# Haiga/nn-with-pytorch-personalized-losses

Hardware: AMD Instinct MI355X
Metric: slates/sec fwd+bwd approxNDCG slate=128 feat=136 (higher is better)
Workload: dtype f32; 1 GPU; approxNDCG + doubleLayerNet (136-136-136-1) train-mode dropout, 100000 queries x slate 128 x 136 feat fp32 per GPU resident in HBM, 25000 slates per GPU per step, one fused launch (fwd+loss+bwd) + grad all-reduce + Adam; queries_per_gpu=100000, slate=128, features=136, batch_per_gpu=25000, net=double, step_windows=4, step_windows_visited=4, last_window_starts_at_float=1305600000, parallelism=query-sharded dp1

## Files before the change

nn-with-pytorch-personalized-losses_amd/csrc/ltr_scorer.hip:

```cpp
#include "../../include/ltr_mi355x.h"
#include "ltr_slate_losses.h"
#include <math.h>
#include <stdlib.h>
#include <string.h>
#include <type_traits>


#ifndef LTR_F16X2
#define LTR_F16X2 0
#endif
#ifndef LTR_LOLO
#define LTR_LOLO 1
#endif

using namespace ltr;

typedef float f32x4 __attribute__((ext_vector_type(4)));

namespace {

constexpr int kTileDocs = 128;
constexpr int kWaves = 8;
constexpr int kThreads = kWaves * 64;
constexpr int kChunkDocs = 64;
// ... 298 lines not shown
                v = __frcp_rn(1.f + __expf(-v))      ;
            }
            if (16 * To + 16 > H) v = (16 * To + 4 * q + r < H) ? v : 0.f;
            h[To][r] = v;
        }
    }
}

template <int ACT>
__device__ __forceinline__ float apply_act_grad(float g, float h) {
    if (ACT == ACT_RELU_DROP) return h > 0.f ? g : 0.f;
    if (ACT == ACT_SIGMOID) return g * (h * (1.f - h));
    return g;
}

template <int NR, int NC, int BH>
__host__ __device__ constexpr int dw_row(int g) { return (g / (NC * BH)) * BH + (g % (NC * BH)) % BH; }
template <int NR, int NC, int BH>
__host__ __device__ constexpr int dw_col(int g) { return (g % (NC * BH)) / BH; }
__host__ __device__ constexpr int dw_count(int NW, int W) {
    const int s = W % (kWaves / 2), simd = NW / (kWaves / 2) + (s < NW % (kWaves / 2) ? 1 : 0);
    return W < kWaves / 2 ? (simd + 1) / 2 : simd / 2;
}
__host__ __device__ constexpr int dw_first(int NW, int W) {
    int g = 0;
    for (int v = 0; v < W; ++v) g += dw_count(NW, v);
    return g;
}
__host__ __device__ constexpr bool dw_sets_balanced(int NW) {
    const int TW = (NW + kWaves - 1) / kWaves;
    int lo = NW, hi = 0;
    for (int s = 0; s < kWaves / 2; ++s) {
        const int t = dw_count(NW, s) + dw_count(NW, s + kWaves / 2);
        lo = t < lo ? t : lo;
        hi = t > hi ? t : hi;
        if (dw_count(NW, s) > TW || dw_count(NW, s + kWaves / 2) > TW) return false;
    }
    return hi - lo <= 1 && dw_first(NW, kWaves) == NW;
}

template <int W, int TW, int NR, int NC, int BH>
struct DwSet {
    static_assert(dw_sets_balanced(NR * NC) && TW == (NR * NC + kWaves - 1) / kWaves, "unbalanced dW tile sets");
    static constexpr int first = dw_first(NR * NC, W), count = dw_count(NR * NC, W);
    static constexpr bool uses_row(int To) {
        for (int j = 0; j < count; ++j)
            if (dw_row<NR, NC, BH>(first + j) == To) return true;
        return false;
    }
    static constexpr bool uses_col(int Ti) {
        for (int j = 0; j < count; ++j)
            if (dw_col<NR, NC, BH>(first + j) == Ti) return true;
        return false;
    }
    static constexpr int n_frags() {
        int n = 0;
        for (int t = 0; t < NR; ++t) n += uses_row(t) ? 1 : 0;
        for (int t = 0; t < NC; ++t) n += uses_col(t) ? 1 : 0;
        return n;
    }
    static constexpr int n_tiles() { return count; }
};

template <int W, int TW, int NR, int NC, int BH, int LD>
__device__ __forceinline__ void dw_load(float (&af)[NR], float (&bf)[NC], const float *ar, const float *br) {
#pragma unroll
    for (int To = 0; To < NR; ++To)
        if (DwSet<W, TW, NR, NC, BH>::uses_row(To)) af[To] = ar[16 * To];
#pragma unroll
    for (int Ti = 0; Ti < NC; ++Ti)
        if (DwSet<W, TW, NR, NC, BH>::uses_col(Ti)) bf[Ti] = br[16 * Ti];
}

template <int W, int TW, int NR, int NC, int BH>
__device__ __forceinline__ void dw_mfma(f32x4 (&acc)[TW], const float (&af)[NR], const float (&bf)[NC]) {
#pragma unroll
    for (int j = 0; j < DwSet<W, TW, NR, NC, BH>::count; ++j) {
        const int g = DwSet<W, TW, NR, NC, BH>::first + j;
        acc[j] = mfma4(af[dw_row<NR, NC, BH>(g)], bf[dw_col<NR, NC, BH>(g)], acc[j]);
    }
}

#ifndef LTR_DW_PIPE
#define LTR_DW_PIPE 0
#endif
#ifndef LTR_PRIO
#define LTR_PRIO 0
#endif
#ifndef LTR_KROT
#define LTR_KROT 0
#endif
#ifndef LTR_H1_BITS
#define LTR_H1_BITS 0
#endif
#ifndef LTR_STG_SWZ
#define LTR_STG_SWZ 0
#endif

template <int W, int TW, int NR, int NC, int BH, int LD>
__device__ __forceinline__ void dw_chunk_w(f32x4 (&acc)[TW], const float *a_base, const float *b_base, const float *a_odd,
                                           const float *b_odd) {
    constexpr int KS = kChunkDocs / 4;
#if LTR_DW_PIPE
    static_assert(!LTR_STG_SWZ, "the pipelined variant reads unswizzled images");
    constexpr int NF = DwSet<W, TW, NR, NC, BH>::n_frags();
    constexpr int NM = DwSet<W, TW, NR, NC, BH>::n_tiles();
    float af0[NR], bf0[NC], af1[NR], bf1[NC];
    dw_load<W, TW, NR, NC, BH, LD>(af0, bf0, a_base, b_base);
#pragma unroll
    for (int s = 0; s < KS; s += 2) {
        dw_load<W, TW, NR, NC, BH, LD>(af1, bf1, a_base + (s + 1) * 4 * LD, b_base + (s + 1) * 4 * LD);
        dw_mfma<W, TW, NR, NC, BH>(acc, af0, bf0);
#pragma unroll
        for (int i = 0; i < (NM > NF ? NM : NF); ++i) {
            if (i < NF) __builtin_amdgcn_sched_group_barrier(0x100, 1, 0);
            if (i < NM) __builtin_amdgcn_sched_group_barrier(0x008, 1, 0);
        }
        if (s + 2 < KS)
            dw_load<W, TW, NR, NC, BH, LD>(af0, bf0, a_base + (s + 2) * 4 * LD, b_base + (s + 2) * 4 * LD);
        dw_mfma<W, TW, NR, NC, BH>(acc, af1, bf1);
#pragma unroll
        for (int i = 0; i < (NM > NF ? NM : NF); ++i) {
            if (i < NF && s + 2 < KS) __builtin_amdgcn_sched_group_barrier(0x100, 1, 0);
            if (i < NM) __builtin_amdgcn_sched_group_barrier(0x008, 1, 0);
        }
    }
#else
    for (int s0 = 0; s0 < KS; ++s0) {
        const int s = LTR_KROT ? ((s0 + (W >= kWaves / 2 ? KS / 2 : 0)) % KS) : s0;
        float af[NR], bf[NC];
        dw_load<W, TW, NR, NC, BH, LD>(af, bf, ((s & 1) ? a_odd : a_base) + s * 4 * LD, ((s & 1) ? b_odd : b_base) + s * 4 * LD);
        dw_mfma<W, TW, NR, NC, BH>(acc, af, bf);
    }
#endif
}

template <int TW, int NR, int NC, int BH, int LD>
__device__ __forceinline__ void dw_chunk(int w, f32x4 (&acc)[TW], const float *a_base, const float *b_base, const float *a_odd = nullptr,
                                         const float *b_odd = nullptr) {
    if (!a_odd) a_odd = a_base;
    if (!b_odd) b_odd = b_base;
    switch (w) {
        case 0: dw_chunk_w<0, TW, NR, NC, BH, LD>(acc, a_base, b_base, a_odd, b_odd); break;
        case 1: dw_chunk_w<1, TW, NR, NC, BH, LD>(acc, a_base, b_base, a_odd, b_odd); break;
        case 2: dw_chunk_w<2, TW, NR, NC, BH, LD>(acc, a_base, b_base, a_odd, b_odd); break;
        case 3: dw_chunk_w<3, TW, NR, NC, BH, LD>(acc, a_base, b_base, a_odd, b_odd); break;
        case 4: dw_chunk_w<4, TW, NR, NC, BH, LD>(acc, a_base, b_base, a_odd, b_odd); break;
        case 5: dw_chunk_w<5, TW, NR, NC, BH, LD>(acc, a_base, b_base, a_odd, b_odd); break;
        case 6: dw_chunk_w<6, TW, NR, NC, BH, LD>(acc, a_base, b_base, a_odd, b_odd); break;
        default: dw_chunk_w<7, TW, NR, NC, BH, LD>(acc, a_base, b_base, a_odd, b_odd); break;
    }
}

#if LTR_F16X2
typedef short s16x4 __attribute__((ext_vector_type(4)));
typedef _Float16 h16x4 __attribute__((ext_vector_type(4)));
typedef unsigned int u32x2 __attribute__((ext_vector_type(2)));

template <int LDH>
__device__ __forceinline__ h16x8 tr_frag_h(const uint16_t *lane_base, int r0, int t) {
    typedef __attribute__((address_space(3))) s16x4 *lp4;
    const uint16_t *p = lane_base + r0 * LDH + 16 * t;
    const s16x4 lo = __builtin_amdgcn_ds_read_tr16_b64_v4i16((lp4)(p));
    const s16x4 hi = __builtin_amdgcn_ds_read_tr16_b64_v4i16((lp4)(p + 16 * LDH));
    const u32x2 l2 = __builtin_bit_cast(u32x2, lo), h2 = __builtin_bit_cast(u32x2, hi);
    return __builtin_bit_cast(h16x8, u32x4{l2[0], l2[1], h2[0], h2[1]});
}

__device__ __forceinline__ void split4(const f32x4 &v, float sc, u32x2 &hi, u32x2 &lo) {
    h16x4 h, l;
#pragma unroll
    for (int r = 0; r < 4; ++r) {
        const float x = v[r] * sc;
        h[r] = (_Float16)x;
        l[r] = (_Float16)(x - (float)h[r]);
    }
    hi = __builtin_bit_cast(u32x2, h);
    lo = __builtin_bit_cast(u32x2, l);
}

template <int W, int TW, int NR, int NC, int BH, int LDH, int KS>
__device__ __forceinline__ void dw_chunk_h_w(f32x4 (&acc)[TW], const uint16_t *ahi, const uint16_t *alo, const uint16_t *bhi,
                                             const uint16_t *blo) {
    using S = DwSet<W, TW, NR, NC, BH>;
#pragma unroll
    for (int s = 0; s < KS; ++s) {
        h16x8 ah[NR], al[NR];
#pragma unroll
        for (int To = 0; To < NR; ++To)
            if (S::uses_row(To)) {
                ah[To] = tr_frag_h<LDH>(ahi, 32 * s, To);
                al[To] = tr_frag_h<LDH>(alo, 32 * s, To);
            }
#pragma unroll
        for (int Ti = 0; Ti < NC; ++Ti)
            if (S::uses_col(Ti)) {
                const h16x8 bh = tr_frag_h<LDH>(bhi, 32 * s, Ti), bl = tr_frag_h<LDH>(blo, 32 * s, Ti);
#pragma unroll
                for (int j = 0; j < S::count; ++j) {
                    const int g = S::first + j;
                    if (dw_col<NR, NC, BH>(g) == Ti) {
                        const int r = dw_row<NR, NC, BH>(g);
                        acc[j] = __builtin_amdgcn_mfma_f32_16x16x32_f16(ah[r], bh, acc[j], 0, 0, 0);
                        acc[j] = __builtin_amdgcn_mfma_f32_16x16x32_f16(ah[r], bl, acc[j], 0, 0, 0);
                        acc[j] = __builtin_amdgcn_mfma_f32_16x16x32_f16(al[r], bh, acc[j], 0, 0, 0);
                        if (LTR_LOLO) acc[j] = __builtin_amdgcn_mfma_f32_16x16x32_f16(al[r], bl, acc[j], 0, 0, 0);
                    }
                }
            }
    }
}

template <int TW, int NR, int NC, int BH, int LDH, int KS>
__device__ __forceinline__ void dw_chunk_h(int w, f32x4 (&acc)[TW], const uint16_t *ahi, const uint16_t *alo, const uint16_t *bhi,
                                           const uint16_t *blo) {
    switch (w) {
        case 0: dw_chunk_h_w<0, TW, NR, NC, BH, LDH, KS>(acc, ahi, alo, bhi, blo); break;
        case 1: dw_chunk_h_w<1, TW, NR, NC, BH, LDH, KS>(acc, ahi, alo, bhi, blo); break;
        case 2: dw_chunk_h_w<2, TW, NR, NC, BH, LDH, KS>(acc, ahi, alo, bhi, blo); break;
        case 3: dw_chunk_h_w<3, TW, NR, NC, BH, LDH, KS>(acc, ahi, alo, bhi, blo); break;
        case 4: dw_chunk_h_w<4, TW, NR, NC, BH, LDH, KS>(acc, ahi, alo, bhi, blo); break;
        case 5: dw_chunk_h_w<5, TW, NR, NC, BH, LDH, KS>(acc, ahi, alo, bhi, blo); break;
        case 6: dw_chunk_h_w<6, TW, NR, NC, BH, LDH, KS>(acc, ahi, alo, bhi, blo); break;
        default: dw_chunk_h_w<7, TW, NR, NC, BH, LDH, KS>(acc, ahi, alo, bhi, blo); break;
    }
}

template <int NT, int KT, int LDH, int NMAX>
__device__ __forceinline__ void gemm_wx_hx(__amdgpu_buffer_rsrc_t rsrc, int base_bytes, int lane_off, const uint16_t *xhi_row,
                                           const uint16_t *xlo_row, f32x4 (&out)[NMAX], float un) {
    constexpr int KP = (KT + 1) / 2;
    constexpr int NSTEP = KP * NT, NLOAD = 2 * NSTEP, R = LTR_RING_H;
    f32x4 ring[R];
#pragma unroll
    for (int n = 0; n < R; ++n)
        if (n < NLOAD) ring[n] = load_frag(rsrc, lane_off, base_bytes + n * 1024);
#pragma unroll
    for (int To = 0; To < NT; ++To) out[To] = f32x4{0.f, 0.f, 0.f, 0.f};
    h16x8 bhi, blo;
#pragma unroll
    for (int n = 0; n < NSTEP; ++n) {
        const int P = n / NT, To = n % NT;
        if (To == 0) {
            const u32x2 z = {0u, 0u};
            const u32x2 h0 = *reinterpret_cast<const u32x2 *>(xhi_row + 32 * P), l0 = *reinterpret_cast<const u32x2 *>(xlo_row + 32 * P);
            const u32x2 h1 = 2 * P + 1 < KT ? *reinterpret_cast<const u32x2 *>(xhi_row + 32 * P + 16) : z;
            const u32x2 l1 = 2 * P + 1 < KT ? *reinterpret_cast<const u32x2 *>(xlo_row + 32 * P + 16) : z;
            bhi = __builtin_bit_cast(h16x8, u32x4{h0[0], h0[1], h1[0], h1[1]});
            blo = __builtin_bit_cast(h16x8, u32x4{l0[0], l0[1], l1[0], l1[1]});
        }
        const h16x8 ahi = __builtin_bit_cast(h16x8, ring[(2 * n) % R]);
        const h16x8 alo = __builtin_bit_cast(h16x8, ring[(2 * n + 1) % R]);
        if (2 * n + R < NLOAD) ring[(2 * n) % R] = load_frag(rsrc, lane_off, base_bytes + (2 * n + R) * 1024);
        if (2 * n + 1 + R < NLOAD) ring[(2 * n + 1) % R] = load_frag(rsrc, lane_off, base_bytes + (2 * n + 1 + R) * 1024);
        out[To] = __builtin_amdgcn_mfma_f32_16x16x32_f16(ahi, bhi, out[To], 0, 0, 0);
        out[To] = __builtin_amdgcn_mfma_f32_16x16x32_f16(ahi, blo, out[To], 0, 0, 0);
        out[To] = __builtin_amdgcn_mfma_f32_16x16x32_f16(alo, bhi, out[To], 0, 0, 0);
        if (LTR_LOLO) out[To] = __builtin_amdgcn_mfma_f32_16x16x32_f16(alo, blo, out[To], 0, 0, 0);
        __builtin_amdgcn_sched_barrier(0);
    }
#pragma unroll
    for (int To = 0; To < NT; ++To) out[To] *= un;
}

__device__ __forceinline__ int grow_exp(int ex, float m) {
    int e = __builtin_amdgcn_frexp_expf(m);
    e = m > 0.f ? e : -100;
    e = e < -100 ? -100 : e;
    return e > ex ? e : ex;
}
#endif

template <int W, int TW, int NR, int NC, int BH>
__device__ __forceinline__ void dw_store_w(const f32x4 (&acc)[TW], float *dst, int q, int d, float scale) {
#pragma unroll
    for (int j = 0; j < DwSet<W, TW, NR, NC, BH>::count; ++j) {
        const int g = DwSet<W, TW, NR, NC, BH>::first + j;
        const int To = dw_row<NR, NC, BH>(g), Ti = dw_col<NR, NC, BH>(g);
#pragma unroll
        for (int r = 0; r < 4; ++r) dst[(16 * To + 4 * q + r) * (NC * 16) + 16 * Ti + d] = acc[j][r] * scale;
    }
}

template <int TW, int NR, int NC, int BH>
__device__ __forceinline__ void dw_store(int w, const f32x4 (&acc)[TW], float *dst, int q, int d, float scale = 1.f) {
    switch (w) {
        case 0: dw_store_w<0, TW, NR, NC, BH>(acc, dst, q, d, scale); break;
        case 1: dw_store_w<1, TW, NR, NC, BH>(acc, dst, q, d, scale); break;
        case 2: dw_store_w<2, TW, NR, NC, BH>(acc, dst, q, d, scale); break;
        case 3: dw_store_w<3, TW, NR, NC, BH>(acc, dst, q, d, scale); break;
        case 4: dw_store_w<4, TW, NR, NC, BH>(acc, dst, q, d, scale); break;
        case 5: dw_store_w<5, TW, NR, NC, BH>(acc, dst, q, d, scale); break;
        case 6: dw_store_w<6, TW, NR, NC, BH>(acc, dst, q, d, scale); break;
        default: dw_store_w<7, TW, NR, NC, BH>(acc, dst, q, d, scale); break;
    }
}

#ifdef LTR_STAMPS
#define LTR_STAMP(k)                                                                                          \
    if (a.stamps && lane == 0 && (st - (int)blockIdx.x) / (int)gridDim.x == a.stamp_tile)                      \
        a.stamps[((size_t)blockIdx.x * kWaves + w) * 16 + (k)] = __builtin_readcyclecounter();
#else
#define LTR_STAMP(k)
#endif

template <class N>
__host__ __device__ constexpr int kXV4() { return (16 * (N::F / 4) + 63) / 64; }

template <class N>
__device__ __forceinline__ void load_x_tile(f32x4 (&xr)[kXV4<N>()], const PipeArgs &a, long long row0, int lane) {
    constexpr int V4_PER_ROW = N::F / 4;
    constexpr int V4 = 16 * V4_PER_ROW;
    const f32x4 *src = reinterpret_cast<const f32x4 *>(a.X + row0 * N::F);
#pragma unroll
    for (int m = 0; m < kXV4<N>(); ++m) {
        const int e = lane + 64 * m;
        f32x4 v = {0.f, 0.f, 0.f, 0.f};
        if (e < V4 && row0 + e / V4_PER_ROW < a.n_docs) v = src[e];
        xr[m] = v;
    }
}

#ifndef LTR_LOSS_UNR
#define LTR_LOSS_UNR 1
#endif
#ifndef LTR_XDMA
#define LTR_XDMA 1
#endif
#ifndef LTR_PIPE_ST128_MAXH
#define LTR_PIPE_ST128_MAXH 64
#endif
#ifndef LTR_PIPE_ST128
#define LTR_PIPE_ST128 1
#endif
#ifndef LTR_X_AUX
#define LTR_X_AUX 2
#endif
template <class N>
__device__ __forceinline__ void dma_x_rows(const PipeArgs &a, float *Xs, long long row0, int w, int lane) {
    typedef __attribute__((address_space(1))) const void *gptr_t;
    typedef __attribute__((address_space(3))) void *lptr_t;
#pragma unroll
    for (int r = 0; r < 16; ++r) {
        float *dst = Xs + (16 * w + r) * N::LD;
        if (row0 + r < a.n_docs) {
            if (lane < N::F / 4)
                __builtin_amdgcn_global_load_lds((gptr_t)(a.X + (row0 + r) * N::F + 4 * lane), (lptr_t)dst, 16, 0, LTR_X_AUX);
        } else if (lane < N::F / 4) {
            *reinterpret_cast<f32x4 *>(dst + 4 * lane) = f32x4{0.f, 0.f, 0.f, 0.f};
        }
    }
}

template <class N, class Stamp>
__device__ __forceinline__ void dw2_chunks(int w, int chunk, int crow, int q, int d, const f32x4 (&dz2)[N::NT2], const f32x4 (&h1)[N::H1T],
                                           f32x4 (&acc)[N::TW2], float *Ds, float *Hs, Stamp stamp) {
    constexpr int LD = N::LD;
#pragma unroll
    for (int c = 0; c < 2; ++c) {
        if (c > 0) __syncthreads();
        if (chunk == c) {
#pragma unroll
            for (int To = 0; To < N::NT2; ++To)
                *reinterpret_cast<f32x4 *>(Ds + crow * LD + 16 * To + ((4 * q) ^ (LTR_STG_SWZ ? 4 * ((crow >> 1) & 3) : 0))) = dz2[To];
#pragma unroll
            for (int T = 0; T < N::H1T; ++T)
                *reinterpret_cast<f32x4 *>(Hs + crow * LD + 16 * T + ((4 * q) ^ (LTR_STG_SWZ ? 4 * ((crow >> 1) & 3) : 0))) = h1[T];
        }
#ifdef LTR_STAMPS_DW
        stamp(c == 0 ? 10 : 13);
#endif
        __syncthreads();
#ifdef LTR_STAMPS_DW
        stamp(c == 0 ? 11 : 14);
#endif
        dw_chunk<N::TW2, N::NT2, N::H1T, N::BH2, LD>(w, acc, Ds + q * LD + (d ^ (LTR_STG_SWZ ? 4 * (q >> 1) : 0)),
                                                     Hs + q * LD + (d ^ (LTR_STG_SWZ ? 4 * (q >> 1) : 0)),
                                                     Ds + q * LD + (d ^ (LTR_STG_SWZ ? 4 * (2 + (q >> 1)) : 0)),
                                                     Hs + q * LD + (d ^ (LTR_STG_SWZ ? 4 * (2 + (q >> 1)) : 0)));
#ifdef LTR_STAMPS_DW
        if (c == 0) stamp(12);
#endif
    }
}

#include "ltr_fcw.h"

template <class N, int MODE, int LOSS, int ST = 0>
__global__ void __launch_bounds__(kThreads, 2) slate_pipeline_kernel(const PipeArgs a) {
    constexpr int LD = N::LD;
    extern __shared__ __attribute__((aligned(16))) float smem[];
    float *Xs = smem;
    float *Ds = Xs + kTileDocs * LD;
    float *Hs = Ds + kChunkDocs * LD;
    float *sc = Hs + kChunkDocs * LD;
    float *yl = sc + kTileDocs;
    float *gn = yl + kTileDocs;
    float *gg = gn + kTileDocs;
    float *dsc = gg + kTileDocs;
    float *uu = dsc + kTileDocs;
    float *mk = uu + kTileDocs;
    float *xt = mk + kTileDocs;
    float *w3s = xt + kTileDocs;
    float *dw3 = w3s + N::NT2 * 16 + 16;
    float *scratch = dw3 + kWaves * N::NT2 * 16;

    const int tid = threadIdx.x;
    const int lane = tid & 63;
    const int w = __builtin_amdgcn_readfirstlane(tid >> 6);
    const int q = lane >> 4, d = lane & 15;

    const __amdgpu_buffer_rsrc_t wrsrc =
        __builtin_amdgcn_make_buffer_rsrc(const_cast<float *>(a.packed), 0, N::PACKED * 4, 0x00020000);
    const int lane_off = lane * 16;

#if LTR_PRIO
    if (w >= kWaves / 2) __builtin_amdgcn_s_setprio(1);
#endif
    for (int j = tid; j < N::NT2 * 16 + 16; j += kThreads) w3s[j] = a.packed[N::W3_OFF + j];
    for (int j = tid; j < kWaves * N::NT2 * 16; j += kThreads) dw3[j] = 0.f;
    for (int j = tid; j < kThreads + 4 * 32; j += kThreads) scratch[j] = 0.f;
    if (MODE == MODE_FUSED && LOSS == 0) {
        __syncthreads();
        ltr_fill_inv_discount(scratch + 256, kTileDocs, tid, kThreads);
    }
    float db3 = 0.f;
    f32x4 accW1[N::TW1], accW2[N::TW2];
    if (MODE != MODE_FWD) {
#pragma unroll
        for (int n = 0; n < N::TW1; ++n) accW1[n] = f32x4{0.f, 0.f, 0.f, 0.f};
#pragma unroll
        for (int n = 0; n < N::TW2; ++n) accW2[n] = f32x4{0.f, 0.f, 0.f, 0.f};
    }
    const int my_row = 16 * w + d;
    const int chunk = w >> 2;
    const int crow = 16 * (w & 3) + d;

    constexpr bool XPREF = x_reg_prefetch<N, MODE>();
    constexpr bool XDMA = LTR_XDMA && !XPREF;
#if LTR_F16X2
#ifndef LTR_DWH
#define LTR_DWH 1
#endif
    constexpr bool DWH = LTR_DWH && MODE != MODE_FWD && (XDMA || XPREF);
    constexpr int LDH = LD;
    uint16_t *Xhi = reinterpret_cast<uint16_t *>(Xs), *Xlo = Xhi + kTileDocs * LDH;
    uint16_t *Sg = reinterpret_cast<uint16_t *>(Ds);
    float *exch = scratch + kThreads + 4 * 32;
    int exx = 1, exh = 1, exd2 = -100, exd1 = -100, E1 = -400, E2 = -400;
    float w3max = 0.f;
#else
    constexpr bool DWH = false;
#endif
#ifndef LTR_REORD
#define LTR_REORD 1
#endif
    constexpr bool REORD = LTR_REORD && XDMA && !N::TWO && !DWH && MODE != MODE_FWD;
    f32x4 xn[kXV4<N>()];
#if LTR_F16X2
    if (DWH) {
        for (int e = tid; e < kTileDocs * (LD - N::F); e += kThreads) {
            const int r = e / (LD - N::F), c = N::F + e % (LD - N::F);
            Xhi[r * LDH + c] = 0;
            Xlo[r * LDH + c] = 0;
        }
        __syncthreads();
        float m = 0.f;
        for (int j = lane; j < N::NT2 * 16; j += 64) m = fmaxf(m, fabsf(w3s[j]));
        w3max = wave_allmax(m);
    } else
#endif
    if (XDMA) {
        constexpr int PADV4 = (LD - N::F) / 4;
        for (int e = tid; e < kTileDocs * PADV4; e += kThreads) {
            const int r = e / PADV4, c4 = e - r * PADV4;
            f32x4 v = {0.f, 0.f, 0.f, 0.f};
            if (c4 == 0) v[0] = 1.f;
            *reinterpret_cast<f32x4 *>(Xs + r * LD + N::F + 4 * c4) = v;
        }
    }
    const int lane_outer = lane;
    for (int st = blockIdx.x; st < a.n_super; st += gridDim.x) {
        const long long doc_base = (long long)st * kTileDocs;
        constexpr bool DEHOIST = N::H1 > 64 && MODE != MODE_FWD;
        int lane = lane_outer;
        if (DEHOIST) asm volatile("" : "+v"(lane));
        const int q = lane >> 4, d = lane & 15;
        const int my_row = 16 * w + d;
        const int crow = 16 * (w & 3) + d;
        const int lane_off = lane * 16;
        const int tid = 64 * w + lane;
#if LTR_F16X2
        auto convert_x = [&]() {
            float xm = 1.f;
#pragma unroll
            for (int i = 0; i < kWaves; ++i) xm = fmaxf(xm, exch[i]);
            exx = grow_exp(exx, xm);
            const float sx = ldexpf(1.f, 14 - exx);
            constexpr int V4_PER_ROW = N::F / 4, V4 = 16 * V4_PER_ROW;
#pragma unroll
            for (int mm = 0; mm < kXV4<N>(); ++mm) {
                const int e = lane + 64 * mm;
                if (e < V4) {
                    u32x2 hi, lo;
                    split4(xn[mm], sx, hi, lo);
                    const int off = (16 * w + e / V4_PER_ROW) * LDH + 4 * (e % V4_PER_ROW);
                    *reinterpret_cast<u32x2 *>(Xhi + off) = hi;
                    *reinterpret_cast<u32x2 *>(Xlo + off) = lo;
                }
            }
            if (lane < 16) {
                Xhi[(16 * w + lane) * LDH + N::F] = __builtin_bit_cast(uint16_t, (_Float16)sx);
                Xlo[(16 * w + lane) * LDH + N::F] = 0;
            }
        };
        auto publish_xmax = [&]() {
            float m = 0.f;
#pragma unroll
            for (int mm = 0; mm < kXV4<N>(); ++mm)
#pragma unroll
                for (int r = 0; r < 4; ++r) m = fmaxf(m, fabsf(xn[mm][r]));
            m = wave_allmax(m);
            if (lane == 0) exch[w] = m;
        };
        if (DWH && XPREF) {
            if (st == (int)blockIdx.x) load_x_tile<N>(xn, a, doc_base + 16 * w, lane);
            publish_xmax();
        }
#endif
// ... 128 lines not shown
                for (int To = 0; To < N::NT2; ++To) h2[To] = h1[To];
            activate<N::A2, N::H2, N::NT2, MODE == MODE_FWD>(h2, q, a, 1, a.keep2, gdoc);
            if (MODE == MODE_FWD && a.acts_out) {
#pragma unroll
                for (int T = 0; T < N::NT2; ++T)
                    *reinterpret_cast<f32x4 *>(a.acts_out + act_base + (size_t)(N::NT1 + T) * 256) = h2[T];
            }
        }
        LTR_STAMP(3)
        {
            float p0 = 0.f;
#pragma unroll
            for (int To = 0; To < N::NT2; ++To) {
                const f32x4 wv = *reinterpret_cast<const f32x4 *>(w3s + 16 * To + 4 * q);
#pragma unroll
                for (int r = 0; r < 4; ++r) p0 += wv[r] * h2[To][r];
            }
            p0 += __shfl_xor(p0, 16, 64);
            p0 += __shfl_xor(p0, 32, 64);
            if (q == 0) sc[my_row] = p0 + w3s[N::NT2 * 16];
        }
        if (MODE == MODE_FWD) {
            __syncthreads();
            if (tid < kTileDocs && doc_base + tid < a.n_docs) a.scores_out[doc_base + tid] = sc[tid];
            continue;
        }
        LTR_STAMP(4)
        if (MODE == MODE_FUSED && LTR_SKIP(a, 1)) {
            __syncthreads();
            if (tid < kTileDocs) dsc[tid] = 1e-3f * sc[tid];
        } else if (MODE == MODE_FUSED) {
            __syncthreads();
            int tl = tid;
            if (DEHOIST) asm volatile("" : "+v"(tl));
            const int S_ = ST ? ST : a.S;
            const int group = 4 * S_;
            const int gid = tl / group;
            const SlateGroup g = make_group(S_, group, scratch + gid * (group + 32), tl);
            const int so = gid * S_;
            const long long slate = (long long)st * (kTileDocs / S_) + gid;
            float loss;
            if (LOSS == 0) {
                auto stamp_fn = [&](int k) { LTR_STAMP(k) };
                auto run = [&](auto s_tag, auto nw_tag, auto stamper) {
                    constexpr int SS = decltype(s_tag)::value, NWS = decltype(nw_tag)::value;
                    const int gi = tl / (64 * NWS), so2 = gi * SS;
                    const float *scp = sc + so2;
                    return approx_ndcg_fused_shared<SS, NWS, false>(tl - gi * 64 * NWS, [&](int j) { return scp[j]; }, sc + so2, yl + so2, gn + so2,
                                                                    gg + so2, uu + so2, xt + so2, mk + so2, scratch + gi * 32, scratch + 256, a.alpha, a.eps,
                                                                    a.gscale, [&](int i, float v) { dsc[so2 + i] = v; }, stamper);
                };
                if constexpr (ST == 128) loss = run(std::integral_constant<int, 128>(), std::integral_constant<int, 8>(), stamp_fn);
                else if (a.S == 128) loss = run(std::integral_constant<int, 128>(), std::integral_constant<int, 8>(), stamp_fn);
                else if (a.S == 64) loss = run(std::integral_constant<int, 64>(), std::integral_constant<int, 4>(), NoStamp());
                else loss = run(std::integral_constant<int, 32>(), std::integral_constant<int, 2>(), NoStamp());
            }
            else if (LOSS == 1)
                loss = listnet_slate(g, yl + so, sc + so, a.apply_sigmoid != 0, a.gscale, true,
                                     [&](int i, float v) { dsc[so + i] = v; });
            else {
                LambdaLds L;
                L.sc = sc + so; L.yl = yl + so; L.gn = gn + so; L.w1 = gg + so; L.invd = uu + so; L.delta = mk + so;
                L.rk = reinterpret_cast<int *>(xt + so);
                float count;
                loss = lambda_slate<-1>(g, L, a.lp, a.gscale, true, &count, [&](int i, float v) { dsc[so + i] = v; });
                if (g.t == 0 && slate < a.B && a.slate_count) a.slate_count[slate] = count;
            }
            if (g.t == 0 && slate < a.B) a.slate_loss[slate] = loss;
        }
        __syncthreads();

        LTR_STAMP(5)
        float pf = 0.f;
        if (!XPREF && !REORD) {
            const long long nb = (long long)(st + gridDim.x) * kTileDocs;
            const long long fl = nb * N::F + (long long)tid * 32;
            if (st + (int)gridDim.x < a.n_super && fl < a.n_docs * N::F) pf = a.X[fl];
            constexpr int LINES = (kTileDocs * N::F + 31) / 32;
            if (tid + kThreads < LINES) {
                const long long fl2 = fl + (long long)kThreads * 32;
                if (st + (int)gridDim.x < a.n_super && fl2 < a.n_docs * N::F) pf += a.X[fl2];
            }
        }
        const float ds0 = gdoc < a.n_docs ? dsc[my_row] : 0.f;
        db3 += wave_allsum((q == 0) ? ds0 : 0.f);
        const float slope = a.dropout ? a.drop_scale : 1.f;
        const float ds2 = (N::A2 == ACT_RELU_DROP) ? ds0 * slope : ds0;
#pragma unroll
        for (int To = 0; To < N::NT2; ++To) {
            const f32x4 wv = *reinterpret_cast<const f32x4 *>(w3s + 16 * To + 4 * q);
            const f32x4 sv = row_sum4_to_lane15(h2[To] * ds0);
#pragma unroll
            for (int r = 0; r < 4; ++r) {
                if (d == 15)
                    __hip_atomic_fetch_add(&dw3[w * N::NT2 * 16 + 16 * To + 4 * q + r], sv[r], __ATOMIC_RELAXED,
                                           __HIP_MEMORY_SCOPE_WORKGROUP);
                h2[To][r] = apply_act_grad<N::A2>(ds2 * wv[r], h2[To][r]);
            }
        }
#if LTR_H1_BITS
        unsigned hbits[(N::NT1 * 4 + 31) / 32] = {};
        if (N::A1 == ACT_RELU_DROP) {
#pragma unroll
            for (int To = 0; To < N::NT1; ++To)
#pragma unroll
                for (int r = 0; r < 4; ++r)
                    hbits[(To * 4 + r) >> 5] |= (h1[To][r] > 0.f ? 1u : 0u) << ((To * 4 + r) & 31);
        }
#endif
        LTR_STAMP(6)
        auto stamp_dw = [&](int k) { LTR_STAMP(k) };
#if LTR_F16X2
        if (DWH && !N::TWO) {
            float hm = 1.f;
#pragma unroll
            for (int i = 0; i < kWaves; ++i) hm = fmaxf(hm, exch[8 + i]);
            exh = grow_exp(exh, hm);
            const float dm = wave_allmax(fmaxf(fabsf(dsc[lane]), fabsf(dsc[lane + 64])));
            exd2 = grow_exp(exd2, dm * slope * w3max);
            if (exd2 + exh != E2) {
                const float f = ldexpf(1.f, E2 - (exd2 + exh));
#pragma unroll
                for (int n = 0; n < N::TW2; ++n) accW2[n] *= f;
                E2 = exd2 + exh;
            }
            const float sd = ldexpf(1.f, 14 - exd2), sh = ldexpf(1.f, 14 - exh);
            const int lb = (4 * q + (d >> 2)) * LDH + 4 * (d & 3);
#pragma unroll
            for (int c = 0; c < 2; ++c) {
                if (c > 0) __syncthreads();
                if (chunk == c) {
#pragma unroll
                    for (int To = 0; To < N::NT2; ++To) {
                        u32x2 hi, lo;
                        split4(h2[To], sd, hi, lo);
                        *reinterpret_cast<u32x2 *>(Sg + crow * LDH + 16 * To + 4 * q) = hi;
                        *reinterpret_cast<u32x2 *>(Sg + (64 + crow) * LDH + 16 * To + 4 * q) = lo;
                    }
#pragma unroll
                    for (int T = 0; T < N::H1T; ++T) {
                        u32x2 hi, lo;
                        split4(h1[T], sh, hi, lo);
                        *reinterpret_cast<u32x2 *>(Sg + (128 + crow) * LDH + 16 * T + 4 * q) = hi;
                        *reinterpret_cast<u32x2 *>(Sg + (192 + crow) * LDH + 16 * T + 4 * q) = lo;
                    }
                }
                __syncthreads();
                dw_chunk_h<N::TW2, N::NT2, N::H1T, N::BH2, LDH, 2>(w, accW2, Sg + lb, Sg + 64 * LDH + lb, Sg + 128 * LDH + lb,
                                                                   Sg + 192 * LDH + lb);
            }
        } else
#endif
        if (!REORD) {
            if (!N::TWO && !LTR_SKIP(a, 2)) dw2_chunks<N>(w, chunk, crow, q, d, h2, h1, accW2, Ds, Hs, stamp_dw);
            LTR_STAMP(7)
        }
        f32x4 dz1[N::NT1];
        if (N::TWO) {
#pragma unroll
            for (int To = 0; To < N::NT1; ++To) dz1[To] = h2[To];
        }
#if LTR_F16X2
        else if (!LTR_SKIP(a, 4)) gemm_wx_h<N::NT1, N::NT2>(wrsrc, N::W2TH_OFF * 4, lane_off, h2, dz1, w3s[N::NT2 * 16 + 6]);
#else
        else if (!LTR_SKIP(a, 4)) gemm_wx<N::NT1, N::NT2>(wrsrc, N::W2T_OFF * 4, lane_off, h2, dz1);
#endif
        else
#pragma unroll
            for (int To = 0; To < N::NT1; ++To) dz1[To] = h2[To < N::NT2 ? To : 0];
#pragma unroll
        for (int To = 0; To < (N::TWO ? 0 : N::NT1); ++To)
#pragma unroll
            for (int r = 0; r < 4; ++r) {
                const float gsc = (N::A1 == ACT_RELU_DROP) ? dz1[To][r] * slope : dz1[To][r];
#if LTR_H1_BITS
                float v = (N::A1 == ACT_RELU_DROP)
                              ? (((hbits[(To * 4 + r) >> 5] >> ((To * 4 + r) & 31)) & 1u) ? gsc : 0.f)
                              : apply_act_grad<N::A1>(gsc, h1[To][r]);
#else
                float v = apply_act_grad<N::A1>(gsc, h1[To][r]);
#endif
                if (16 * To + 16 > N::H1) v = (16 * To + 4 * q + r < N::H1) ? v : 0.f;
                dz1[To][r] = v;
            }
        if (REORD) { LTR_STAMP(7) } else { LTR_STAMP(8) }
#if LTR_F16X2
        if (DWH) {
            float m = 0.f;
#pragma unroll
            for (int To = 0; To < N::NT1; ++To)
#pragma unroll
                for (int r = 0; r < 4; ++r) m = fmaxf(m, fabsf(dz1[To][r]));
            m = wave_allmax(m);
            if (lane == 0) exch[16 + w] = m;
            __syncthreads();
            float dm = 0.f;
#pragma unroll
            for (int i = 0; i < kWaves; ++i) dm = fmaxf(dm, exch[16 + i]);
            exd1 = grow_exp(exd1, dm);
            if (exd1 + exx != E1) {
                const float f = ldexpf(1.f, E1 - (exd1 + exx));
#pragma unroll
                for (int n = 0; n < N::TW1; ++n) accW1[n] *= f;
                E1 = exd1 + exx;
            }
            const float sd = ldexpf(1.f, 14 - exd1);
#pragma unroll
            for (int To = 0; To < N::NT1; ++To) {
                u32x2 hi, lo;
                split4(dz1[To], sd, hi, lo);
                *reinterpret_cast<u32x2 *>(Sg + my_row * LDH + 16 * To + 4 * q) = hi;
                *reinterpret_cast<u32x2 *>(Sg + (128 + my_row) * LDH + 16 * To + 4 * q) = lo;
            }
            __syncthreads();
            if (XPREF && st + (int)gridDim.x < a.n_super)
                load_x_tile<N>(xn, a, (long long)(st + gridDim.x) * kTileDocs + 16 * w, lane);
            const int lb = (4 * q + (d >> 2)) * LDH + 4 * (d & 3);
            dw_chunk_h<N::TW1, N::NT1, N::XT, N::BH1, LDH, 4>(w, accW1, Sg + lb, Sg + 128 * LDH + lb, Xhi + lb, Xlo + lb);
        } else {
#endif
        if (MODE != MODE_FWD && XPREF && st + (int)gridDim.x < a.n_super)
            load_x_tile<N>(xn, a, (long long)(st + gridDim.x) * kTileDocs + 16 * w, lane);
#ifndef LTR_DW1_SINGLE
#define LTR_DW1_SINGLE 1
#endif
        if (N::H1 <= 64 || LTR_DW1_SINGLE) {
            if (!REORD) __syncthreads();
#pragma unroll
            for (int To = 0; To < N::NT1; ++To)
                *reinterpret_cast<f32x4 *>(Ds + my_row * LD + 16 * To + ((4 * q) ^ (LTR_STG_SWZ ? 4 * ((my_row >> 1) & 3) : 0))) = dz1[To];
            __syncthreads();
            if (!LTR_SKIP(a, 2)) {
#pragma unroll
                for (int c = 0; c < 2; ++c)
                    dw_chunk<N::TW1, N::NT1, N::XT, N::BH1, LD>(w, accW1, Ds + (64 * c + q) * LD + (d ^ (LTR_STG_SWZ ? 4 * (q >> 1) : 0)),
                                                                Xs + (64 * c + q) * LD + d,
                                                                Ds + (64 * c + q) * LD + (d ^ (LTR_STG_SWZ ? 4 * (2 + (q >> 1)) : 0)),
                                                                Xs + (64 * c + q) * LD + d);
            }
        } else {
#pragma unroll
            for (int c = 0; c < 2; ++c) {
                __syncthreads();
                if (chunk == c) {
#pragma unroll
                    for (int To = 0; To < N::NT1; ++To)
                        *reinterpret_cast<f32x4 *>(Ds + crow * LD + 16 * To + ((4 * q) ^ (LTR_STG_SWZ ? 4 * ((crow >> 1) & 3) : 0))) = dz1[To];
                }
                __syncthreads();
                if (!LTR_SKIP(a, 2))
                    dw_chunk<N::TW1, N::NT1, N::XT, N::BH1, LD>(w, accW1, Ds + q * LD + (d ^ (LTR_STG_SWZ ? 4 * (q >> 1) : 0)),
                                                                Xs + (64 * c + q) * LD + d,
                                                                Ds + q * LD + (d ^ (LTR_STG_SWZ ? 4 * (2 + (q >> 1)) : 0)),
                                                                Xs + (64 * c + q) * LD + d);
            }
        }
        if (REORD) {
            LTR_STAMP(8)
            __syncthreads();
            if (st + (int)gridDim.x < a.n_super) dma_x_rows<N>(a, Xs, (long long)(st + gridDim.x) * kTileDocs + 16 * w, w, lane);
            if (!LTR_SKIP(a, 2)) dw2_chunks<N>(w, chunk, crow, q, d, h2, h1, accW2, Ds, Hs, stamp_dw);
        }
#if LTR_F16X2
        }
#endif
        LTR_STAMP(9)
        asm volatile("" ::"v"(pf));
    }

    if (MODE == MODE_FWD) return;
    float *part = a.partials + (size_t)blockIdx.x * N::PART;
#if LTR_F16X2
    const float us1 = DWH ? ldexpf(1.f, E1 - 28) : 1.f, us2 = DWH ? ldexpf(1.f, E2 - 28) : 1.f;
#else
    const float us1 = 1.f, us2 = 1.f;
#endif
    dw_store<N::TW1, N::NT1, N::XT, N::BH1>(w, accW1, part + N::P_W1, q, d, us1);
    if (!N::TWO) dw_store<N::TW2, N::NT2, N::H1T, N::BH2>(w, accW2, part + N::P_W2, q, d, us2);
    __syncthreads();
    for (int j = tid; j < N::NT2 * 16; j += kThreads) {
        float s = 0.f;
        for (int ww = 0; ww < kWaves; ++ww) s += dw3[ww * N::NT2 * 16 + j];
        part[N::P_W3 + j] = s;
    }
    if (lane == 0) scratch[w] = db3;
    __syncthreads();
    if (tid == 0) {
        float s = 0.f;
        for (int ww = 0; ww < kWaves; ++ww) s += scratch[ww];
        part[N::P_B3] = s;
    }
}


__global__ void dropout_mask_kernel(unsigned long long seed, int layer, long long n_docs, int H, unsigned thr16, uint8_t *out) {
    const long long e = ltr_block_id() * blockDim.x + threadIdx.x;
    if (e >= n_docs * H) return;
    const long long doc = e / H;
    const int n = (int)(e - doc * H);
    if (thr16) out[e] = ((keep_word(seed, layer + 2, doc, n >> 1) >> (16 * (n & 1))) & 0xffffu) >= thr16 ? 1 : 0;
    else out[e] = (keep_word(seed, layer, doc, n >> 5) >> (n & 31)) & 1u;
}

static inline void decode_dropout(int dropout, int &on, unsigned &thr16, float &scale) {
    on = dropout & 1;
    unsigned bits = (unsigned)dropout & ~1u;
    float p = 0.5f;
    if (bits) memcpy(&p, &bits, sizeof p);
    if (!(p > 0.f)) on = 0;
    if (!(p < 1.f)) p = 0.5f;
    thr16 = p == 0.5f ? 0u : (unsigned)(p * 65536.f + 0.5f);
    if (thr16 > 65535u) thr16 = 65535u;
    scale = 1.f / (1.f - p);
}

template <class N>
__global__ void pack_kernel(const float *__restrict__ W1, const float *__restrict__ b1, const float *__restrict__ W2,
                            const float *__restrict__ b2, const float *__restrict__ w3, const float *__restrict__ b3,
                            float *__restrict__ packed, int Fr, int H1r, int H2r) {
    const int gt = blockIdx.x * blockDim.x + threadIdx.x;
    const int stride = gridDim.x * blockDim.x;
    auto w1aug = [&](int n, int f) { return n < H1r ? (f < Fr ? W1[n * Fr + f] : (f == N::F ? b1[n] : 0.f)) : 0.f; };
    auto w2aug = [&](int n, int f) { return n < H2r ? (f < H1r ? W2[n * H1r + f] : (f == N::H1 ? b2[n] : 0.f)) : 0.f; };
    for (int e = gt; e < N::NT1 * N::XT * 256; e += stride) {
        const int s = e & 3, lane = (e >> 2) & 63, tile = e >> 8, To = tile / N::XT, T = tile - To * N::XT;
        packed[N::W1F_OFF + e] = w1aug(16 * To + (lane & 15), 16 * T + 4 * (lane >> 4) + s);
    }
    for (int e = gt; e < (N::TWO ? 0 : N::NT2 * N::H1T * 256); e += stride) {
        const int s = e & 3, lane = (e >> 2) & 63, tile = e >> 8, To = tile / N::H1T, T = tile - To * N::H1T;
        packed[N::W2F_OFF + e] = w2aug(16 * To + (lane & 15), 16 * T + 4 * (lane >> 4) + s);
    }
    for (int e = gt; e < (N::TWO ? 0 : N::NT1 * N::NT2 * 256); e += stride) {
        const int s = e & 3, lane = (e >> 2) & 63, tile = e >> 8, Ti = tile / N::NT2, T = tile - Ti * N::NT2;
        const int in = 16 * Ti + (lane & 15), o = 16 * T + 4 * (lane >> 4) + s;
        packed[N::W2T_OFF + e] = (o < H2r && in < H1r) ? W2[o * H1r + in] : 0.f;
    }
#if LTR_F16X2
    __shared__ float red[3][256];
    float mx[3] = {0.f, 0.f, 0.f};
    for (int e = threadIdx.x; e < N::H1 * (N::F + 1); e += blockDim.x) mx[0] = fmaxf(mx[0], fabsf(w1aug(e / (N::F + 1), e % (N::F + 1))));
    for (int e = threadIdx.x; e < (N::TWO ? 0 : N::H2 * (N::H1 + 1)); e += blockDim.x) {
        const float v = fabsf(w2aug(e / (N::H1 + 1), e % (N::H1 + 1)));
        mx[1] = fmaxf(mx[1], v);
        if (e % (N::H1 + 1) < N::H1) mx[2] = fmaxf(mx[2], v);
    }
    for (int k = 0; k < 3; ++k) red[k][threadIdx.x] = mx[k];
    __syncthreads();
    for (int o = 128; o > 0; o >>= 1) {
        if ((int)threadIdx.x < o)
            for (int k = 0; k < 3; ++k) red[k][threadIdx.x] = fmaxf(red[k][threadIdx.x], red[k][threadIdx.x + o]);
        __syncthreads();
    }
    float scl[3], inv[3];
    for (int k = 0; k < 3; ++k) {
        int ex = __builtin_amdgcn_frexp_expf(red[k][0]);
        ex = ex < -100 ? -100 : ex;
        scl[k] = ldexpf(1.f, 14 - ex);
        inv[k] = ldexpf(1.f, ex - 14);
    }
    uint16_t *ph = reinterpret_cast<uint16_t *>(packed);
    auto put = [&](size_t off_halfs, int hh, float v) {
        const _Float16 hi = (_Float16)v;
        const _Float16 out = ((hh >> 9) & 1) ? (_Float16)(v - (float)hi) : hi;
        ph[off_halfs + hh] = __builtin_bit_cast(uint16_t, out);
    };
    auto geom = [](int hh, int NT, int &To, int &i, int &f) {
        const int j = hh & 7, lane = (hh >> 3) & 63, step = hh >> 10, P = step / NT;
        To = step % NT;
        i = lane & 15;
        f = 32 * P + 16 * (j >> 2) + 4 * (lane >> 4) + (j & 3);
    };
    for (int hh = gt; hh < N::KP1 * N::NT1 * 1024; hh += stride) {
        int To, i, f;
        geom(hh, N::NT1, To, i, f);
        put((size_t)N::W1H_OFF * 2, hh, w1aug(16 * To + i, f) * scl[0]);
    }
    for (int hh = gt; hh < (N::TWO ? 0 : N::KP2 * N::NT2 * 1024); hh += stride) {
        int To, i, f;
        geom(hh, N::NT2, To, i, f);
        put((size_t)N::W2H_OFF * 2, hh, w2aug(16 * To + i, f) * scl[1]);
    }
    for (int hh = gt; hh < (N::TWO ? 0 : N::KPT * N::NT1 * 1024); hh += stride) {
        int Ti, i, o;
        geom(hh, N::NT1, Ti, i, o);
        const int in = 16 * Ti + i;
        put((size_t)N::W2TH_OFF * 2, hh, (o < H2r && in < H1r) ? W2[o * H1r + in] * scl[2] : 0.f);
    }
    for (int hh = gt; hh < (N::TWO ? N::KP1 * N::NT1 * 1024 : 0); hh += stride) {
        const int j = hh & 7, lane = (hh >> 3) & 63, step = hh >> 10, tile = step / N::KP1, P = step % N::KP1;
        put((size_t)N::W1B_OFF * 2, hh, w1aug(16 * tile + (lane & 15), 32 * P + 8 * (lane >> 4) + j) * scl[0]);
    }
#endif
    for (int e = gt; e < N::NT2 * 16 + 16; e += stride) {
        float v = e < H2r ? w3[e] : (e == N::NT2 * 16 ? b3[0] : 0.f);
#if LTR_F16X2
        if (e >= N::NT2 * 16 + 4 && e < N::NT2 * 16 + 7) v = inv[e - N::NT2 * 16 - 4];
#endif
        packed[N::W3_OFF + e] = v;
    }
}


constexpr int kTrH1 = 64, kTrH2 = 32;
__global__ void triple_fold_kernel(const float *__restrict__ W1, const float *__restrict__ b1, const float *__restrict__ W2,
                                   const float *__restrict__ b2, const float *__restrict__ w3, int kTrF, int copies,
                                   float *__restrict__ W1e, float *__restrict__ b1e, float *__restrict__ w3e) {
    const int e = blockIdx.x * blockDim.x + threadIdx.x;
    if (e >= kTrH2 * (kTrF + 1)) return;
    const int u = e / (kTrF + 1), f = e % (kTrF + 1);
    double acc = 0.0;
    if (f < kTrF) {
        for (int k = 0; k < kTrH1; ++k) acc += (double)W2[u * kTrH1 + k] * (double)W1[k * kTrF + f];
        for (int c = 0; c < copies; ++c) W1e[(c * kTrH2 + u) * kTrF + f] = (float)acc;
    } else {
// ... 398 lines not shown
```

Before: 4.154 million slates/s.

## Stage dW operands in unit-major swizzled LDS layout for weight-gradient MFMAs

Adds a unit-major (hidden unit rows, doc columns, XOR-swizzled) LDS staging layout for dz1, dz2 and h1, plus a new dw_um routine that reads A/B fragments as contiguous f32x4 along the doc dimension. It is used in the REORD path for both dW2 chunks and the single-pass dW1, replacing row-major staging with per-element scalar LDS stores. The aim is fewer LDS read instructions and bank conflicts in the weight-gradient MFMA loops. The cost is scalar scatter writes on staging, and a strided scalar read path for the X operand.

```diff
diff --git a/nn-with-pytorch-personalized-losses_amd/csrc/ltr_scorer.hip b/nn-with-pytorch-personalized-losses_amd/csrc/ltr_scorer.hip
--- a/nn-with-pytorch-personalized-losses_amd/csrc/ltr_scorer.hip
+++ b/nn-with-pytorch-personalized-losses_amd/csrc/ltr_scorer.hip
@@ -474,6 +474,64 @@
     }
 }
 
+template <int RS>
+__device__ __forceinline__ int um_off(int u, int c) { return u * RS + 4 * ((c >> 2) ^ (u & 15)) + (c & 3); }
+__device__ __forceinline__ int um_dz1_col(int c) { return (c & ~15) + 4 * (c & 3) + ((c >> 2) & 3); }
+
+template <int W, int TW, int NR, int NC, int BH, int RS, int LDB, int G, bool BX>
+__device__ __forceinline__ void dw_um_w(f32x4 (&acc)[TW], const float *A, const float *B, int q, int d) {
+    using S = DwSet<W, TW, NR, NC, BH>;
+    const int v = q ^ d;
+    const float *ar = A + d * RS;
+    const float *br = BX ? B + q * LDB + d : B + d * RS;
+    constexpr auto run_len = [](int t) {
+        const int c = dw_col<NR, NC, BH>(S::first + t);
+        if (t > 0 && dw_col<NR, NC, BH>(S::first + t - 1) == c) return 0;
+        int n = 1;
+        while (t + n < S::count && dw_col<NR, NC, BH>(S::first + t + n) == c) ++n;
+        return n;
+    };
+#pragma unroll 1
+    for (int g = 0; g < G; ++g) {
+        const int o = 64 * (g >> 2) + 4 * ((4 * (g & 3)) ^ v);
+#pragma unroll
+        for (int t = 0; t < S::count; ++t) {
+            const int n = run_len(t);
+            if (n == 0) continue;
+            const int Ti = dw_col<NR, NC, BH>(S::first + t);
+            f32x4 bfr, afr[BH];
+            if (BX) {
+#pragma unroll
+                for (int j = 0; j < 4; ++j) bfr[j] = br[(16 * g + 4 * j) * LDB + 16 * Ti];
+            } else {
+                bfr = *reinterpret_cast<const f32x4 *>(br + 16 * Ti * RS + o);
+            }
+#pragma unroll
+            for (int k = 0; k < BH; ++k)
+                if (k < n) afr[k] = *reinterpret_cast<const f32x4 *>(ar + 16 * dw_row<NR, NC, BH>(S::first + t + k) * RS + o);
+#pragma unroll
+            for (int j = 0; j < 4; ++j)
+#pragma unroll
+                for (int k = 0; k < BH; ++k)
+                    if (k < n) acc[t + k] = mfma4(afr[k][j], bfr[j], acc[t + k]);
+        }
+    }
+}
+
+template <int TW, int NR, int NC, int BH, int RS, int LDB, int G, bool BX>
+__device__ __forceinline__ void dw_um(int w, f32x4 (&acc)[TW], const float *A, const float *B, int q, int d) {
+    switch (w) {
+        case 0: dw_um_w<0, TW, NR, NC, BH, RS, LDB, G, BX>(acc, A, B, q, d); break;
+        case 1: dw_um_w<1, TW, NR, NC, BH, RS, LDB, G, BX>(acc, A, B, q, d); break;
+        case 2: dw_um_w<2, TW, NR, NC, BH, RS, LDB, G, BX>(acc, A, B, q, d); break;
+        case 3: dw_um_w<3, TW, NR, NC, BH, RS, LDB, G, BX>(acc, A, B, q, d); break;
+        case 4: dw_um_w<4, TW, NR, NC, BH, RS, LDB, G, BX>(acc, A, B, q, d); break;
+        case 5: dw_um_w<5, TW, NR, NC, BH, RS, LDB, G, BX>(acc, A, B, q, d); break;
+        case 6: dw_um_w<6, TW, NR, NC, BH, RS, LDB, G, BX>(acc, A, B, q, d); break;
+        default: dw_um_w<7, TW, NR, NC, BH, RS, LDB, G, BX>(acc, A, B, q, d); break;
+    }
+}
+
 #if LTR_F16X2
 typedef short s16x4 __attribute__((ext_vector_type(4)));
 typedef _Float16 h16x4 __attribute__((ext_vector_type(4)));
@@ -674,14 +732,24 @@
     }
 }
 
-template <class N, class Stamp>
+template <class N, bool UM, class Stamp>
 __device__ __forceinline__ void dw2_chunks(int w, int chunk, int crow, int q, int d, const f32x4 (&dz2)[N::NT2], const f32x4 (&h1)[N::H1T],
                                            f32x4 (&acc)[N::TW2], float *Ds, float *Hs, Stamp stamp) {
     constexpr int LD = N::LD;
+    static_assert(!UM || (N::NT2 * 16 <= LD && N::H1T * 16 <= LD), "unit-major chunk images must fit the [64][LD] staging buffers");
 #pragma unroll
     for (int c = 0; c < 2; ++c) {
         if (c > 0) __syncthreads();
-        if (chunk == c) {
+        if (UM && chunk == c) {
+#pragma unroll
+            for (int To = 0; To < N::NT2; ++To)
+#pragma unroll
+                for (int r = 0; r < 4; ++r) Ds[um_off<kChunkDocs>(16 * To + 4 * q + r, crow)] = dz2[To][r];
+#pragma unroll
+            for (int T = 0; T < N::H1T; ++T)
+#pragma unroll
+                for (int r = 0; r < 4; ++r) Hs[um_off<kChunkDocs>(16 * T + 4 * q + r, crow)] = h1[T][r];
+        } else if (chunk == c) {
 #pragma unroll
             for (int To = 0; To < N::NT2; ++To)
                 *reinterpret_cast<f32x4 *>(Ds + crow * LD + 16 * To + ((4 * q) ^ (LTR_STG_SWZ ? 4 * ((crow >> 1) & 3) : 0))) = dz2[To];
@@ -696,7 +764,10 @@
 #ifdef LTR_STAMPS_DW
         stamp(c == 0 ? 11 : 14);
 #endif
-        dw_chunk<N::TW2, N::NT2, N::H1T, N::BH2, LD>(w, acc, Ds + q * LD + (d ^ (LTR_STG_SWZ ? 4 * (q >> 1) : 0)),
+        if constexpr (UM)
+            dw_um<N::TW2, N::NT2, N::H1T, N::BH2, kChunkDocs, LD, kChunkDocs / 16, false>(w, acc, Ds, Hs, q, d);
+        else
+            dw_chunk<N::TW2, N::NT2, N::H1T, N::BH2, LD>(w, acc, Ds + q * LD + (d ^ (LTR_STG_SWZ ? 4 * (q >> 1) : 0)),
                                                      Hs + q * LD + (d ^ (LTR_STG_SWZ ? 4 * (q >> 1) : 0)),
                                                      Ds + q * LD + (d ^ (LTR_STG_SWZ ? 4 * (2 + (q >> 1)) : 0)),
                                                      Hs + q * LD + (d ^ (LTR_STG_SWZ ? 4 * (2 + (q >> 1)) : 0)));
@@ -1131,7 +1202,7 @@
         } else
 #endif
         if (!REORD) {
-            if (!N::TWO && !LTR_SKIP(a, 2)) dw2_chunks<N>(w, chunk, crow, q, d, h2, h1, accW2, Ds, Hs, stamp_dw);
+            if (!N::TWO && !LTR_SKIP(a, 2)) dw2_chunks<N, false>(w, chunk, crow, q, d, h2, h1, accW2, Ds, Hs, stamp_dw);
             LTR_STAMP(7)
         }
         f32x4 dz1[N::NT1];
@@ -1200,16 +1271,30 @@
 #endif
         if (MODE != MODE_FWD && XPREF && st + (int)gridDim.x < a.n_super)
             load_x_tile<N>(xn, a, (long long)(st + gridDim.x) * kTileDocs + 16 * w, lane);
+#ifndef LTR_DW1_UM
+#define LTR_DW1_UM 1
+#endif
 #ifndef LTR_DW1_SINGLE
 #define LTR_DW1_SINGLE 1
 #endif
         if (N::H1 <= 64 || LTR_DW1_SINGLE) {
             if (!REORD) __syncthreads();
-#pragma unroll
-            for (int To = 0; To < N::NT1; ++To)
-                *reinterpret_cast<f32x4 *>(Ds + my_row * LD + 16 * To + ((4 * q) ^ (LTR_STG_SWZ ? 4 * ((my_row >> 1) & 3) : 0))) = dz1[To];
+            if constexpr (REORD && LTR_DW1_UM) {
+                static_assert(N::NT1 * 16 <= LD, "the unit-major dz1 image must fit the [128][LD] staging region");
+                const int col = um_dz1_col(my_row);
+#pragma unroll
+                for (int To = 0; To < N::NT1; ++To)
+#pragma unroll
+                    for (int r = 0; r < 4; ++r) Ds[um_off<kTileDocs>(16 * To + 4 * q + r, col)] = dz1[To][r];
+            } else {
+#pragma unroll
+                for (int To = 0; To < N::NT1; ++To)
+                    *reinterpret_cast<f32x4 *>(Ds + my_row * LD + 16 * To + ((4 * q) ^ (LTR_STG_SWZ ? 4 * ((my_row >> 1) & 3) : 0))) = dz1[To];
+            }
             __syncthreads();
-            if (!LTR_SKIP(a, 2)) {
+            if constexpr (REORD && LTR_DW1_UM) {
+                if (!LTR_SKIP(a, 2)) dw_um<N::TW1, N::NT1, N::XT, N::BH1, kTileDocs, LD, kTileDocs / 16, true>(w, accW1, Ds, Xs, q, d);
+            } else if (!LTR_SKIP(a, 2)) {
 #pragma unroll
                 for (int c = 0; c < 2; ++c)
                     dw_chunk<N::TW1, N::NT1, N::XT, N::BH1, LD>(w, accW1, Ds + (64 * c + q) * LD + (d ^ (LTR_STG_SWZ ? 4 * (q >> 1) : 0)),
@@ -1238,7 +1323,7 @@
             LTR_STAMP(8)
             __syncthreads();
             if (st + (int)gridDim.x < a.n_super) dma_x_rows<N>(a, Xs, (long long)(st + gridDim.x) * kTileDocs + 16 * w, w, lane);
-            if (!LTR_SKIP(a, 2)) dw2_chunks<N>(w, chunk, crow, q, d, h2, h1, accW2, Ds, Hs, stamp_dw);
+            if (!LTR_SKIP(a, 2)) dw2_chunks<N, true>(w, chunk, crow, q, d, h2, h1, accW2, Ds, Hs, stamp_dw);
         }
 #if LTR_F16X2
         }
```

Result: slower. 3.740 million slates/s (median of 2 runs) (-10.0%).
